# fernandezdaniel/MOBOCMF

Hardware: AMD Instinct MI355X
Metric: ELBO steps/sec (MFDGP d=8 M=512 N=8192 S=8) (higher is better)
Workload: dtype f64

## Files before the change

include/mobocmf_hip.h:

```cpp
#ifndef MOBOCMF_HIP_H
#define MOBOCMF_HIP_H

#include <stddef.h>
#include <stdint.h>

#ifdef __cplusplus
extern "C" {
#endif

typedef void* mobocmf_stream_t;

#define MOBOCMF_MAX_D 32
#define MOBOCMF_MAX_XDIV 48

enum {
    MOBOCMF_OK = 0,
    MOBOCMF_BAD_ARG = 1,
    MOBOCMF_WORKSPACE_TOO_SMALL = 2,
    MOBOCMF_HIP_ERROR = 3,
    MOBOCMF_NOT_PD = 4,
    MOBOCMF_BAD_ARCH = 5
};

typedef struct mobocmf_tuning {
    uint32_t struct_size;
    int32_t small_gemm_max;
    int32_t small_panel_max;
    int32_t tile_rows;
    int32_t pair_mode;
    int32_t mid_gemm_max;
    int32_t mid_gemm_waves;
    int32_t syrk_workgroups;
    int32_t sparse_backward;
    int32_t potrf_cols;
} mobocmf_tuning;
int mobocmf_tuning_init(mobocmf_tuning* t);

typedef struct {
    int32_t kind;
    int32_t d;
    int32_t M;
    int32_t xdiv;
    int64_t Np;
    int32_t branch;
    int32_t want_dx;
    double jitter;
    double min_var;
    int32_t params_const;
    int32_t reserved;
    const mobocmf_tuning* tuning;
    void* const* probe_events;
} mobocmf_layer_desc;
#define MOBOCMF_PROBE_EVENTS 11


int mobocmf_version(void);
int mobocmf_device_arch_ok(void);

int mobocmf_layer_workspace_bytes(const mobocmf_layer_desc* desc, size_t* saved_bytes, size_t* scratch_bytes);

int mobocmf_layer_forward(const mobocmf_layer_desc* desc, const double* x, const double* f, const double* Zx,
                          const double* zf, const double* hyp, const double* m, const double* L_S ,
                          double* mean, double* var, double* kl, int32_t* info, void* saved, size_t saved_bytes,
                          void* scratch, size_t scratch_bytes, mobocmf_stream_t stream);

int mobocmf_layer_backward(const mobocmf_layer_desc* desc, const double* x, const double* f, const double* Zx,
                           const double* zf, const double* hyp, const double* m, const double* L_S,
// ... 402 lines not shown
```

mobocmf_amd/_lib.py:

```python
import ctypes
import os

_HERE = os.path.dirname(os.path.abspath(__file__))
LIB_PATH = os.environ.get("MOBOCMF_HIP_LIB") or os.path.join(_HERE, "csrc", "libmobocmf_hip.so")

OK, BAD_ARG, WORKSPACE_TOO_SMALL, HIP_ERROR, NOT_PD, BAD_ARCH = range(6)
_ERR = {1: "MOBOCMF_BAD_ARG", 2: "MOBOCMF_WORKSPACE_TOO_SMALL", 3: "MOBOCMF_HIP_ERROR", 4: "MOBOCMF_NOT_PD",
        5: "MOBOCMF_BAD_ARCH"}


class Tuning(ctypes.Structure):
    _fields_ = [("struct_size", ctypes.c_uint32), ("small_gemm_max", ctypes.c_int32), ("small_panel_max", ctypes.c_int32),
                ("tile_rows", ctypes.c_int32), ("pair_mode", ctypes.c_int32), ("mid_gemm_max", ctypes.c_int32),
                ("mid_gemm_waves", ctypes.c_int32), ("syrk_workgroups", ctypes.c_int32), ("sparse_backward", ctypes.c_int32),
                ("potrf_cols", ctypes.c_int32)]
    KNOBS = tuple(n for n, _ in _fields_[1:])

    def copy(self):
        t = Tuning()
        ctypes.memmove(ctypes.byref(t), ctypes.byref(self), ctypes.sizeof(Tuning))
        return t


PROBE_EVENTS = 11


class LayerDesc(ctypes.Structure):
    _fields_ = [("kind", ctypes.c_int32), ("d", ctypes.c_int32), ("M", ctypes.c_int32), ("xdiv", ctypes.c_int32),
                ("Np", ctypes.c_int64), ("branch", ctypes.c_int32), ("want_dx", ctypes.c_int32),
                ("jitter", ctypes.c_double), ("min_var", ctypes.c_double), ("params_const", ctypes.c_int32),
                ("reserved", ctypes.c_int32), ("tuning", ctypes.POINTER(Tuning)), ("probe_events", ctypes.c_void_p)]


TINY_MAX_LAYERS, TINY_MAX_M, TINY_MAX_D = 3, 32, 8
COOP_MAX_M = 128
FROZEN_MAX_M = 512
FROZEN_SPLIT_MAX_M = 1024
STEP_GRADIENTS, STEP_UPDATE, STEP_FORWARD, STEP_INPUT_GRADIENTS, STEP_COUPLED = range(5)
STEP_CHAIN_VALID = 16


class TinyModel(ctypes.Structure):
    _L = TINY_MAX_LAYERS
    _fields_ = [("L", ctypes.c_int32), ("M", ctypes.c_int32), ("d", ctypes.c_int32), ("S", ctypes.c_int32),
                ("N", ctypes.c_int32), ("rows", ctypes.c_int32 * _L), ("trainable", ctypes.c_uint32 * _L),
                ("branch", ctypes.c_int32),
                ("x", ctypes.c_void_p), ("y", ctypes.c_void_p), ("fid", ctypes.c_void_p), ("Zx", ctypes.c_void_p),
                ("raw", (ctypes.c_void_p * 7) * _L), ("m", ctypes.c_void_p * _L), ("L_S", ctypes.c_void_p * _L),
                ("raw_noise", ctypes.c_void_p * _L), ("noise_lo", ctypes.c_double * _L), ("noise_hi", ctypes.c_double * _L),
# ... 229 lines not shown
```

mobocmf_amd/csrc/api.hip:

```cpp
#include "common.h"

static const mobocmf_tuning kDefaultTuning = {(uint32_t)sizeof(mobocmf_tuning), 384, 512, 0, 0, 1024, 32, 0, 1, 0};
static thread_local const mobocmf_tuning* t_tuning = nullptr;
static thread_local void* const* t_probe = nullptr;
const mobocmf_tuning& tune() { return t_tuning ? *t_tuning : kDefaultTuning; }
bool tuning_ok(const mobocmf_tuning* t) {
    if (!t) return true;
    return t->struct_size == sizeof(mobocmf_tuning) && t->small_gemm_max >= 1 && t->small_gemm_max <= 512 &&
           t->small_panel_max >= 1 && t->small_panel_max <= 512 && (t->tile_rows == 0 || t->tile_rows == 64 || t->tile_rows == 128) &&
           t->pair_mode >= 0 && t->pair_mode <= 2 && t->mid_gemm_max >= 0 && t->mid_gemm_max <= 4096 &&
           (t->mid_gemm_waves == 4 || t->mid_gemm_waves == 8 || t->mid_gemm_waves == 32) &&
           (t->syrk_workgroups == 0 || (t->syrk_workgroups >= 16 && t->syrk_workgroups <= 4096)) &&
           (t->sparse_backward == 0 || t->sparse_backward == 1) && (t->potrf_cols == 0 || t->potrf_cols == 1 || t->potrf_cols == 4);
}
TuneScope::TuneScope(const mobocmf_tuning* t, void* const* probe) : prev_t(t_tuning), prev_p(t_probe) {
    t_tuning = t;
    t_probe = probe;
}
TuneScope::~TuneScope() {
    t_tuning = prev_t;
    t_probe = prev_p;
}
void probe_at(int i, hipStream_t s) {
    if (t_probe && i < MOBOCMF_PROBE_EVENTS && t_probe[i]) (void)hipEventRecord((hipEvent_t)t_probe[i], s);
}
static void set_pairing(GemmArgs& g) { g.pair_mode = tune().pair_mode; }
static int panel_tile_rows(int, int64_t) { return tune().tile_rows; }

#define TRY(x)              \
    do {                    \
        int _rc = (x);      \
        if (_rc) return _rc; \
    } while (0)

namespace {

struct Bump {
    uintptr_t base;
    size_t off, cap;
    bool ok;
    Bump(void* p, size_t c) : base((uintptr_t)p), off(0), cap(c), ok(true) {}
    double* take(int64_t n) {
        size_t bytes = ((size_t)n * sizeof(double) + 255) & ~(size_t)255;
        if (bytes > cap || off > cap - bytes) { ok = false; off += bytes; return nullptr; }
        double* r = base ? (double*)(base + off) : nullptr;
        off += bytes;
// ... 137 lines not shown
    S.a = b.take(D.Mp); S.mp = b.take(D.Mp);
}
void carve_panel_saved(Bump& b, const Dims& D, PanelSaved& S) {
    int64_t mn = (int64_t)D.Mp * D.Np;
    S.A = b.take(mn); S.C = b.take(mn);
    S.knn = b.take(D.Np); S.q = b.take(D.Np); S.r = b.take(D.Np); S.varraw = b.take(D.Np);
}
void carve_chain_fwd(Bump& b, const Dims& D, ChainWs& S) {
    S.Dinv = b.take((int64_t)(D.Mp / NB) * NB * NB);
    S.Ld = b.take((int64_t)(D.Mp / NB) * NB * NB);
    S.T = b.take((int64_t)D.Mp * D.Mp);
    S.ws_elems = (int64_t)16 * D.Mp * D.Mp;
    S.ws = b.take(S.ws_elems);
    S.klpart = b.take(D.Mp);
}
void carve_panel_fwd(Bump& b, const Dims& D, PanelFwd& S) {
    S.K = b.take((int64_t)D.Mp * D.Np);
    S.qpart = b.take((int64_t)4 * D.nrb * D.Np);
    S.mupart = b.take((int64_t)4 * D.nrb * D.Np);
    S.rpart = b.take((int64_t)4 * D.nrb * D.Np);
}
void carve_chain_bwd_in(Bump& b, const Dims& D, ChainWs& S) {
    int64_t mm = (int64_t)D.Mp * D.Mp;
    S.H = b.take(mm); S.Hc = b.take(mm); S.da = b.take(D.Mp);
}
void carve_chain_bwd(Bump& b, const Dims& D, ChainWs& S) {
    int64_t mm = (int64_t)D.Mp * D.Mp;
    for (int i = 0; i < 8; ++i) S.W[i] = b.take(mm);
    S.da_tot = b.take(D.Mp);
    S.hyp_part2 = b.take((int64_t)D.ggrid_mm.x * D.ggrid_mm.y * hyp_len(1, MOBOCMF_MAX_D));
    S.df_part2 = b.take((int64_t)D.ggrid_mm.y * D.Mp);
    S.dzf_part2 = b.take((int64_t)D.ggrid_mm.x * D.Mp);
}
void carve_panel_bwd(Bump& b, const Dims& D, const mobocmf_layer_desc* d, PanelBwd& S) {
    int64_t mm = (int64_t)D.Mp * D.Mp, mn = (int64_t)D.Mp * D.Np;
    S.gmu = b.take(D.Np); S.gv = b.take(D.Np); S.gv2 = b.take(D.Np); S.cgv = b.take(D.Np);
    S.blkact = (int32_t*)b.take((D.Np / TILE + 1) / 2);
    S.nclamped = (int32_t*)b.take(4);
    S.dA = b.take(mn); S.dK = b.take(mn);
    S.slab_elems = syrk_slab_elems(D.Mp, D.Np);
    S.slabs = b.take(S.slab_elems);
    S.slabs2 = d->branch == 0 ? b.take(S.slab_elems) : nullptr;
    S.dapart = b.take((D.Np <= 8192 ? D.Np / 16 : D.Np / 64) * (int64_t)D.Mp);
    S.hyp_part = b.take((int64_t)D.ggrid_mn.x * D.ggrid_mn.y * D.H);
    S.df_part = S.dzf_part = nullptr;
    if (d->kind == 1) {
        S.df_part = b.take((int64_t)D.ggrid_mn.y * D.Np);
        S.dzf_part = b.take((int64_t)D.ggrid_mn.x * D.Mp);
    }
    S.dx_part = d->want_dx ? b.take((int64_t)D.ggrid_mn.y * D.nbase * d->d) : nullptr;
}

bool carve_single_saved(void* saved, size_t bytes, const Dims& D, ChainWs& c, PanelSaved& p, size_t* used = nullptr) {
    Bump b(saved, bytes);
    carve_chain_state(b, D, c);
    carve_panel_saved(b, D, p);
    if (used) *used = b.off;
    return b.ok;
}
bool carve_single_fwd(void* scratch, size_t bytes, const Dims& D, ChainWs& c, PanelFwd& p, size_t* used = nullptr) {
    Bump b(scratch, bytes);
    carve_chain_fwd(b, D, c);
    carve_panel_fwd(b, D, p);
    if (used) *used = b.off;
    return b.ok;
}
bool carve_single_bwd(void* scratch, size_t bytes, const Dims& D, const mobocmf_layer_desc* d, ChainWs& c, PanelBwd& p,
                      size_t* used = nullptr) {
    Bump b(scratch, bytes);
    carve_panel_bwd(b, D, d, p);
    carve_chain_bwd_in(b, D, c);
    carve_chain_bwd(b, D, c);
    c.slabs = p.slabs;
    c.slab_elems = p.slab_elems;
    if (used) *used = b.off;
    return b.ok;
}
// ... 97 lines not shown
    return MOBOCMF_OK;
}

int panel_backward(const mobocmf_layer_desc* desc, const Dims& D, const ChainWs& c, const PanelSaved& P, const PanelBwd& B,
                   const double* x, const double* f, const double* Zx, const double* zf, const double* hyp, const double* g_mean,
                   const double* g_var, double* g_f, double* g_zf, double* g_hyp, double* g_x, hipStream_t s) {
    const int Mp = D.Mp;
    const int64_t Np = D.Np, mm = (int64_t)Mp * Mp;
    int32_t* nclamped = c.nclamped ? c.nclamped : B.nclamped;
    double* Hc = desc->branch != 0 ? c.H : c.Hc;
    const int32_t* act = tune().sparse_backward ? B.blkact : nullptr;
    TRY(launch_moments_bwd_prep(g_mean, g_var, P.knn, P.q, P.varraw, desc->branch, desc->min_var, D.N, Np, B.gmu, B.gv,
                                B.gv2, B.cgv, nclamped, c.nclamped ? 1 : 0, (int32_t*)act, s));
    int da_parts = 0;
    {
        GemmArgs ga = gemm_args(c.U, Mp, P.C, Np, B.dA, Np, Mp, Np, Mp, TRI_LOWER_A, 2.0);
        ga.bscale = B.gv; ga.epi = EPI_DA; ga.avec = c.a; ga.gmu = B.gmu; ga.cgv = B.cgv; ga.Aaux = P.A;
        ga.Kreal = D.M;
        ga.rowdot_part = desc->params_const ? nullptr : B.dapart;
        ga.colact = act;
        ga.rm = panel_tile_rows(Mp, Np);
        set_pairing(ga);
        probe_at(3, s);
        TRY(launch_gemm(ga, false, 1, s));
        probe_at(4, s);
        da_parts = desc->params_const ? 0 : gemm_rowdot_parts(ga);
    }
    if (!desc->params_const) {
        probe_at(5, s);
        if (desc->branch == 0) TRY(weighted_syrk_pair(P.A, Np, B.gv, B.cgv, Mp, Np, B.slabs, B.slabs2, c.H, Hc, nclamped, act, s));
        else TRY(weighted_syrk(P.A, Np, B.gv, Mp, Np, B.slabs, c.H, nullptr, nullptr, act, s));
        probe_at(6, s);
    }
    {
        GemmArgs ga = gemm_args(c.LinvT, Mp, B.dA, Np, B.dK, Np, Mp, Np, Mp, TRI_UPPER_A, 1.0);
        ga.Kreal = D.M;
        ga.rm = panel_tile_rows(Mp, Np);
        set_pairing(ga);
        ga.colact = act;
        probe_at(7, s);
        TRY(launch_gemm(ga, false, 1, s));
        probe_at(8, s);
    }
    GramArgs g = {};
    g.kind = desc->kind; g.d = desc->d; g.zdiv = 1; g.Zx = Zx; g.zf = zf; g.M = D.M; g.hyp = hyp; g.Mp = Mp;
    g.xdiv = desc->xdiv; g.x = x; g.f = f; g.nbase = D.nbase;
    g.ldk = Np; g.Np = Np; g.G = B.dK; g.gknn = B.cgv; g.colact = act;
    g.hyp_part = B.hyp_part; g.df_part = B.df_part; g.dzf_part = B.dzf_part; g.dx_part = B.dx_part;
    TRY(launch_gram_bwd(g, desc->want_dx != 0, s));
    probe_at(10, s);
    SumTask tk[5];
    int nt = 0;
    if (da_parts > 0) tk[nt++] = {B.dapart, da_parts, Mp, nullptr, 0, 0, c.da, Mp, 0};
    tk[nt++] = {B.hyp_part, (int64_t)D.ggrid_mn.x * D.ggrid_mn.y, D.H, nullptr, 0, 0, g_hyp, D.H, 0};
    if (desc->kind == 1) {
        tk[nt++] = {B.df_part, D.ggrid_mn.y, Np, nullptr, 0, 0, g_f, D.N, 0};
        tk[nt++] = {B.dzf_part, D.ggrid_mn.x, Mp, nullptr, 0, 0, g_zf, D.M, 0};
    }
    if (desc->want_dx)
        tk[nt++] = {B.dx_part, D.ggrid_mn.y, D.nbase * desc->d, nullptr, 0, 0, g_x, D.nbase * desc->d, 0};
    return launch_sum_partials_multi(tk, nt, s);
}

int chain_backward(int n, const ChainWs& c, int64_t zs, const ChainIO& io, const Dims& D, const bool* zero, const int* acc,
                   const bool* fold, hipStream_t s) {
    const int Mp = D.Mp;
    const int64_t mm = (int64_t)Mp * Mp;
    double *G1 = c.W[0], *G2 = c.W[1], *X = c.W[2], *dU = c.W[3], *Y = c.W[4], *T1 = c.W[5], *T2 = c.W[6], *LT = c.W[7];
    double *dL = G1, *T4 = G2, *Gm = X;
    bool any_clamp_branch = false;
    for (int z = 0; z < n; ++z) {
        if (zero[z]) {
            TRY(launch_zero32(c.H + z * zs, mm * 2, s));
            TRY(launch_zero32(c.Hc + z * zs, mm * 2, s));
            TRY(launch_zero32(c.da + z * zs, (int64_t)Mp * 2, s));
        }
        any_clamp_branch = any_clamp_branch || io.desc[z]->branch == 0;
    }
    for (int z = 0; z < n; ++z)
        if (io.desc[z]->branch != 0 && !zero[z] && (n > 1 || any_clamp_branch))
            TRY(launch_copy_block(c.H + z * zs, Mp, c.Hc + z * zs, Mp, Mp, Mp, s));
    const double* Hc = (n == 1 && io.desc[0]->branch != 0) ? c.H : c.Hc;
    {
        GemmArgs g1 = gemm_args(c.UT, Mp, c.H, Mp, G1, Mp, Mp, Mp, Mp, TRI_UPPER_A, 1.0);
        g1.Kreal = D.M;
        TRY(chain_gemm(g1, false, c, n, zs, s));
        GemmArgs g2 = gemm_args(c.U, Mp, G1, Mp, G2, Mp, Mp, Mp, Mp, TRI_LOWER_A, 1.0);
// ... 748 lines not shown
```

mobocmf_amd/csrc/common.h:

```cpp
#pragma once
#include <hip/hip_runtime.h>
#include <stdint.h>

#include "../../include/mobocmf_hip.h"

#define TILE 128
#define NB 64

static inline int64_t round_up(int64_t v, int64_t m) { return (v + m - 1) / m * m; }

#define HIP_TRY(expr)                                   \
    do {                                                \
        hipError_t _e = (expr);                         \
        if (_e != hipSuccess) return MOBOCMF_HIP_ERROR; \
    } while (0)

const mobocmf_tuning& tune();
bool tuning_ok(const mobocmf_tuning* t);
void probe_at(int i, hipStream_t s);
struct TuneScope {
    const mobocmf_tuning* prev_t;
    void* const* prev_p;
    explicit TuneScope(const mobocmf_tuning* t, void* const* probe = nullptr);
    ~TuneScope();
    TuneScope(const TuneScope&) = delete;
    TuneScope& operator=(const TuneScope&) = delete;
};

enum { TRI_NONE = 0, TRI_LOWER_A = 1, TRI_UPPER_A = 2, TRI_LOWER_B = 4, TRI_UPPER_B = 8 };
enum { EPI_STORE = 0, EPI_COLSTATS = 1, EPI_DA = 2 };

struct GemmArgs {
    const double* A;
    const double* B;
    double* C;
    int64_t lda, ldb, ldc;
    int Mr;
    int64_t Nc;
    int64_t Kd;
    int tri;
    int lower_out;
    int sym_out;
    int sym_full;
    int splitk_diag;
    double alpha;
    int accumulate;
    int rm;
    int pair_mode;
    int64_t slab_stride;
    int64_t strideA, strideB, strideC;
    int batched;
    int zlayers;
    int64_t zsA, zsB, zsC;
    const double* bscale;
    int64_t Kreal;
    double* rowdot_part;
    int stream_out;
    const int32_t* skip_if_zero;
    const int32_t* dual_flag;
    const double* bscale2;
    double* C2;
    const int32_t* colact;
    const int32_t* kact;
    int epi;
    double* colsq_part;
    double* coldot_part;
    const double* avec;
    const double* gmu;
    const double* cgv;
    const double* Aaux;
};

int launch_gemm(const GemmArgs& g, bool B_T, int splitk, hipStream_t s);
int gemm_nt_slabs(const GemmArgs& g, int splitk);
bool gemm_nt_is_small(const GemmArgs& g);
int gemm_rowdot_parts(const GemmArgs& g);
int gemm_colstat_rows(const GemmArgs& g);
int launch_gemm_auto(const GemmArgs& g, bool B_T, double* ws, int64_t ws_elems, hipStream_t s);
int launch_gemm_auto_pair(const GemmArgs& a, const GemmArgs& b, double* ws, int64_t ws_elems, hipStream_t s);

#define MAX_ZL 4

struct GramArgs {
    int kind, d, xdiv, zdiv;
    const double* x;
    const double* f;
    int64_t nbase;
    const double* Zx;
    const double* zf;
    int M;
    const double* hyp;
    double* K;
    int64_t ldk;
    int Mp;
    int64_t Np;
    double* knn;
    double jitter;
    int is_kmm;
    int gm;
    const double* G;
    const double* gknn;
    double* hyp_part;
    double* df_part;
    double* dzf_part;
    double* dx_part;
    const int32_t* colact;
};
int launch_gram_fwd(const GramArgs& g, hipStream_t s);
int launch_gram_bwd(const GramArgs& g, bool want_dx, hipStream_t s);
void gram_grid(const GramArgs& g, dim3* grid);
// ... 97 lines not shown
```

mobocmf_amd/csrc/gemm_f64.hip:

```cpp
#include "common.h"
#include <type_traits>
#include <atomic>

typedef double v4f64 __attribute__((ext_vector_type(4)));
typedef double v2f64 __attribute__((ext_vector_type(2)));

#define BM 128
#define BN 128
#define BK 16
#define KL_MAX 1024
#define TILE_ELEMS (BM * BK)

#define IMG_SWZ(row) ((((row) >> 1) & 1) | ((((row) >> 3) & 1) << 2))


template <int CTRL>
__device__ __forceinline__ double dpp_mov(double v) {
    int lo = __double2loint(v), hi = __double2hiint(v);
    lo = __builtin_amdgcn_update_dpp(0, lo, CTRL, 0xF, 0xF, false);
    hi = __builtin_amdgcn_update_dpp(0, hi, CTRL, 0xF, 0xF, false);
    return __hiloint2double(hi, lo);
}
__device__ __forceinline__ double row16_sum(double v) {
    v += dpp_mov<0xB1>(v);
// ... 146 lines not shown
    const double* B = g.B;
    double* C = g.C;
    if (g.batched) {
        const int zl = g.zlayers > 1 ? z % g.zlayers : 0;
        const int zb = g.zlayers > 1 ? z / g.zlayers : z;
        A += zb * g.strideA + zl * g.zsA;
        B += zb * g.strideB + zl * g.zsB;
        C += zb * g.strideC + zl * g.zsC;
    }
    if (!g.batched && splitk > 1) {
        C += z * g.slab_stride;
        if (g.zlayers > 1) {
            A += blockIdx.z * g.zsA;
            B += blockIdx.z * g.zsB;
            C += blockIdx.z * g.zsC;
        }
    }
    const int nparts = (pair && rb != nrb - 1 - rb) ? 2 : 1;
    const int rb_first = rb;

    const int tid = threadIdx.x;
    const int lane = tid & 63;
    const int wave = __builtin_amdgcn_readfirstlane(tid >> 6);
    const int wr = wave >> 1, wc = wave & 1;
    const int li = lane & 15, lk = lane >> 4;

    if constexpr (!B_T) {
        if (g.colact && g.colact[cb] == 0) {
            if (EPI == EPI_DA && g.rowdot_part) {
                for (int part = 0; part < nparts; ++part) {
                    const int rbp = part == 0 ? rb_first : nrb - 1 - rb_first;
                    for (int i = tid; i < 2 * RM; i += 256)
                        g.rowdot_part[((int64_t)cb * 2 + i / RM) * g.Mr + (int64_t)rbp * RM + i % RM] = 0.0;
                }
            }
            return;
        }
    }

    const int a_row = tid >> 3;
    const int a_lchk = (tid & 7) ^ IMG_SWZ(a_row);
    const double* Ag0 = A + (int64_t)a_row * g.lda + a_lchk * 2;
    const double* Bg = B_T ? B + (cb * BN + a_row) * g.ldb + a_lchk * 2
                           : B + (int64_t)wave * g.ldb + cb * BN;
    auto stage = [&](const double* Ag, int64_t k, int buf) {
        double* As = lds + buf * STAGE_ELEMS;
        double* Bs = As + A_ELEMS;
#pragma unroll
        for (int r = 0; r < RM / 32; ++r) glds16(Ag + (int64_t)(32 * r) * g.lda + k, As + (r * 4 + wave) * 128);
        if (B_T) {
#pragma unroll
            for (int r = 0; r < 4; ++r) glds16(Bg + (int64_t)(32 * r) * g.ldb + k, Bs + (r * 4 + wave) * 128);
        } else {
#pragma unroll
            for (int r = 0; r < 4; ++r)
                glds16(Bg + (k + 4 * r) * g.ldb + lane * 2, Bs + (r * 4 + wave) * 128);
        }
    };

    const int swA = IMG_SWZ(li);
    const int colP0 = ((2 * lk + 0) ^ swA) << 1, colP1 = ((2 * lk + 1) ^ swA) << 1;
    const int a_base = (wr * 16 + li) * BK;
    const int bt_base = (wc * 16 + li) * BK;
    const int bn_base = (4 * lk) * BN + wc * 64 + 2 * li;

  STEP_STAMPS_DECL
// ... 211 lines not shown
        bool done = false;
        if constexpr (B_T) {
            if (g.sym_out && g.lower_out && rb == cb) {
                const int wave_u = __builtin_amdgcn_readfirstlane(wave);
                if (wave_u == 1) {
                    STAGE_LOOP(0, nk, 0, KSTEP_LT)
                } else {
                    STAGE_LOOP(0, nk, 0, KSTEP_LE)
                }
                done = true;
            }
        }
        if (!done) { STAGE_LOOP(0, nk, 0, KSTEP_STD(MMA_ALL)) }
    }
#undef STAGE_LOOP
#undef KSTEP
#undef KOFF
#undef KSTEP_STD
#undef STAGE_NEXT
#undef KSTEP_LE
#undef KSTEP_LT
#undef MMA_IF
#undef MMA_ALL
#undef LOAD_A16
#undef LOAD_B16
#undef MMA16

    STAMP(4 + 4 * part);

    const int64_t row0 = (int64_t)rb * RM + wr * 16 + lk;
    const int64_t col0 = cb * BN + (B_T ? wc * 16 + li : wc * 64 + 2 * li);
    const int ccol = B_T ? wc * 16 + li : wc * 64 + 2 * li;
#define COLOFF(nt) (B_T ? (nt) * 32 : ((nt) >> 1) * 32 + ((nt) & 1))
    if (EPI == EPI_DA && !B_T) {
        v2f64 gm[2], cg[2], cs[2];
#pragma unroll
        for (int h = 0; h < 2; ++h) {
            gm[h] = *(const v2f64*)(g.gmu + col0 + 32 * h);
            cg[h] = *(const v2f64*)(g.cgv + col0 + 32 * h);
            cs[h] = (v2f64){1.0, 1.0};
        }
        if (g.bscale) {
#pragma unroll
            for (int h = 0; h < 2; ++h) cs[h] = *(const v2f64*)(g.bscale + col0 + 32 * h);
        }
        double rdkeep = 0.0;
#pragma unroll
        for (int mt = 0; mt < MT; ++mt) {
            v2f64 av[2][4];
            double ar[4];
#pragma unroll
            for (int r = 0; r < 4; ++r) {
                ar[r] = g.avec[row0 + mt * 32 + 4 * r];
#pragma unroll
                for (int h = 0; h < 2; ++h)
                    av[h][r] = *(const v2f64*)(g.Aaux + (row0 + mt * 32 + 4 * r) * g.ldc + col0 + 32 * h);
            }
#pragma unroll
            for (int r = 0; r < 4; ++r) {
                double rd = 0.0;
#pragma unroll
                for (int h = 0; h < 2; ++h) {
                    const v2f64 a = av[h][r];
                    v2f64 o;
                    o[0] = g.alpha * cs[h][0] * acc[mt][2 * h][r] + ar[r] * gm[h][0] - 2.0 * a[0] * cg[h][0];
                    o[1] = g.alpha * cs[h][1] * acc[mt][2 * h + 1][r] + ar[r] * gm[h][1] - 2.0 * a[1] * cg[h][1];
// ... 96 lines not shown
    if (part == 0) STAMP(13);

#undef COLOFF
    STAMP(9 + part);
  }
  STEP_STAMPS_FLUSH;
}

static bool small_panel_ok(const GemmArgs& g, bool B_T, int splitk);
template <int EPI> static int launch_small_panel(const GemmArgs& g, hipStream_t s);
static bool small_gemm_ok(const GemmArgs& g, bool B_T);
static int launch_small_gemm(const GemmArgs& g, bool B_T, hipStream_t s);

static int tile_rows(const GemmArgs& g, bool B_T, int splitk) {
    if (B_T || splitk > 1 || g.batched || g.lower_out || g.zlayers > 1) return BM;
    if (g.rm == 64 || g.rm == BM) return g.rm;
    if (!(g.tri & (TRI_LOWER_A | TRI_UPPER_A))) return BM;
    const int64_t pairs128 = (int64_t)((g.Mr / BM + 1) / 2) * (g.Nc / BN);
    return pairs128 >= 512 ? BM : 64;
}

int launch_gemm(const GemmArgs& g0, bool B_T, int splitk, hipStream_t s) {
    GemmArgs g = g0;
    if (g.Mr % BM || g.Nc % 16 || g.Kd % BK) return MOBOCMF_BAD_ARG;
    if (B_T || g.batched || splitk > 1) g.colact = nullptr;
    if (g.kact) {
        const int sk_min = (g.lower_out && g.splitk_diag > 0 && g.splitk_diag < splitk) ? g.splitk_diag : splitk;
        const int64_t nb = g.Kd / 128;
        if (!B_T || g.batched || splitk <= 1 || g.zlayers > 1 || g.Kd % 128 || (g.tri & (TRI_LOWER_B | TRI_UPPER_B)) ||
            (nb + sk_min - 1) / sk_min + 2 > KL_MAX)
            g.kact = nullptr;
    }
    if (!B_T && ((g.ldc & 1) || ((uintptr_t)g.C & 15))) return MOBOCMF_BAD_ARG;
    if (small_panel_ok(g, B_T, splitk)) {
        if (g.epi == EPI_COLSTATS) return launch_small_panel<EPI_COLSTATS>(g, s);
        if (g.epi == EPI_DA) return launch_small_panel<EPI_DA>(g, s);
        return launch_small_panel<EPI_STORE>(g, s);
    }
    if (g.Nc % BN) return MOBOCMF_BAD_ARG;
    if (B_T && splitk <= 1 && small_gemm_ok(g, true)) return launch_small_gemm(g, true, s);
    if (!B_T && g.batched > 1 && splitk <= 1 && small_gemm_ok(g, false)) return launch_small_gemm(g, false, s);
    const int rm = tile_rows(g, B_T, splitk);
    int nrb = g.Mr / rm;
    int64_t ncb = g.Nc / BN;
    dim3 grid;
    int pair = 0;
    if (g.batched) {
        grid = dim3((unsigned)(nrb * ncb), 1, (unsigned)(g.batched * (g.zlayers > 1 ? g.zlayers : 1)));
        splitk = 1;
    } else if (splitk > 1) {
        int64_t ntile = g.lower_out ? (int64_t)nrb * (nrb + 1) / 2 : (int64_t)nrb * ncb;
        if (g.lower_out && g.splitk_diag > 0) ntile = 0;
        const int64_t nblk = ntile ? ntile * splitk : (int64_t)nrb * (nrb - 1) / 2 * splitk + (int64_t)nrb * g.splitk_diag;
        grid = dim3((unsigned)(g.dual_flag ? 2 * nblk : nblk), 1, (unsigned)(g.zlayers > 1 ? g.zlayers : 1));
    } else {
        const bool can_pair = (g.tri & (TRI_LOWER_A | TRI_UPPER_A)) && !g.lower_out && nrb > 1;
        if (rm == 64) pair = (can_pair && (int64_t)(nrb / 2) * ncb >= 256) ? 1 : 0;
        else pair = (can_pair && (int64_t)nrb * ncb > 512) ? 1 : 0;
        if (g.pair_mode == 1) pair = 0;
        if (g.pair_mode == 2 && (g.tri & (TRI_LOWER_A | TRI_UPPER_A)) && !g.lower_out && nrb > 1) pair = 1;
        grid = dim3((unsigned)((pair ? (nrb + 1) / 2 : nrb) * ncb), 1, 1);
        splitk = 1;
    }
    const bool tri = (g.tri & (TRI_LOWER_A | TRI_UPPER_A)) != 0 || g.epi == EPI_STORE;
#define LAUNCH(BT, TR, EP, RM_) hipLaunchKernelGGL((gemm_f64_kernel<BT, TR, EP, RM_>), grid, dim3(256), 0, s, g, nrb, ncb, splitk, pair)
    if (B_T) {
        if (g.epi != EPI_STORE) return MOBOCMF_BAD_ARG;
        LAUNCH(true, false, EPI_STORE, 128);
    } else if (rm == 64) {
        if (g.epi == EPI_COLSTATS) LAUNCH(false, true, EPI_COLSTATS, 64);
        else if (g.epi == EPI_DA) LAUNCH(false, true, EPI_DA, 64);
        else LAUNCH(false, true, EPI_STORE, 64);
    } else if (tri) {
        if (g.epi == EPI_COLSTATS) LAUNCH(false, true, EPI_COLSTATS, 128);
        else if (g.epi == EPI_DA) LAUNCH(false, true, EPI_DA, 128);
        else LAUNCH(false, true, EPI_STORE, 128);
    } else {
        if (g.epi == EPI_COLSTATS) LAUNCH(false, false, EPI_COLSTATS, 128);
        else if (g.epi == EPI_DA) LAUNCH(false, false, EPI_DA, 128);
        else LAUNCH(false, false, EPI_STORE, 128);
    }
#undef LAUNCH
    return hipGetLastError() == hipSuccess ? MOBOCMF_OK : MOBOCMF_HIP_ERROR;
}

int gemm_colstat_rows(const GemmArgs& g) {
    if (small_panel_ok(g, false, 1)) return 2 * (g.Mr / BM);
    return 2 * (g.Mr / tile_rows(g, false, 1));
}

__global__ void reduce_slabs_kernel(const double* slabs, int64_t slab_stride, int nslab, double* out, int64_t ld,
                                    int rows, int64_t cols, double scale, int lower_only, int tril, int accumulate,
                                    int64_t zs_slabs, int64_t zs_out) {
    int64_t idx = (int64_t)blockIdx.x * blockDim.x + threadIdx.x;
    if (idx >= (int64_t)rows * cols) return;
    slabs += blockIdx.z * zs_slabs;
    out += blockIdx.z * zs_out;
    int i = (int)(idx / cols);
    int64_t j = idx % cols;
    if (lower_only && (j / TILE) > (i / TILE)) {
        if (tril && !accumulate) out[(int64_t)i * ld + j] = 0.0;
        return;
    }
    double v = 0.0;
    const double* p = slabs + (int64_t)i * cols + j;
    for (int z = 0; z < nslab; ++z) v += p[z * slab_stride];
    v *= scale;
    if (tril && j > i) v = 0.0;
    if (accumulate) v += out[(int64_t)i * ld + j];
    out[(int64_t)i * ld + j] = v;
}

static int small_gemm_limit() { return tune().small_gemm_max; }
static int small_panel_limit() { return tune().small_panel_max; }
template <bool B_T>
__device__ __forceinline__ void small_gemm_body(GemmArgs g, const int bz) {
    constexpr int KC = 128;
    __shared__ double As[16][KC + 1], Bs[KC][17];
    if (g.skip_if_zero && *g.skip_if_zero == 0) return;
    const int tx = threadIdx.x & 15, ty = threadIdx.x >> 4;
    const int64_t r0 = (int64_t)blockIdx.y * 16, c0 = (int64_t)blockIdx.x * 16;
    const bool sym_full = B_T && g.sym_full;
// ... 689 lines not shown
```

mobocmf_amd/functional.py:

```python
import contextlib
import ctypes
import os
import threading

import torch

from . import _lib
from ._lib import LayerDesc

JITTER = 1e-6
MIN_VARIANCE = 1e-10

_scratch = {}


def _stream():
    return ctypes.c_void_p(torch.cuda.current_stream().cuda_stream)


def _ptr(t):
    return ctypes.c_void_p(0 if t is None else t.data_ptr())


def _prep(t):
# ... 52 lines not shown
def release_scratch(stream=None):
    if stream is None:
        _scratch.clear()
        return
    for key in [k for k in _scratch if k[1] == stream.cuda_stream]:
        del _scratch[key]


def hyp_len(kind, d):
    return 1 + d if kind == 0 else 5 + 2 * d


_TUNING_DEFAULT = None
_tuning_tls = threading.local()


def _default_tuning():
    global _TUNING_DEFAULT
    if _TUNING_DEFAULT is None:
        t = _lib.Tuning()
        _lib.check(_lib.load().mobocmf_tuning_init(ctypes.byref(t)), "mobocmf_tuning_init")
        _TUNING_DEFAULT = t
    return _TUNING_DEFAULT


def current_tuning():
    t = getattr(_tuning_tls, "override", None)
    return (t if t is not None else _default_tuning()).copy()


def _set_default(**kw):
    t = _default_tuning()
    for k, v in kw.items():
        assert k in _lib.Tuning.KNOBS, k
        setattr(t, k, int(v))


@contextlib.contextmanager
def tuning(**kw):
    prev = getattr(_tuning_tls, "override", None)
    t = current_tuning()
    for k, v in kw.items():
        if k not in _lib.Tuning.KNOBS:
            raise TypeError("unknown tuning knob %r" % k)
        setattr(t, k, int(v))
    _tuning_tls.override = t
    try:
        yield t
    finally:
        _tuning_tls.override = prev


_probe_tls = threading.local()


@contextlib.contextmanager
def probe_events(table, layer=None):
    prev = getattr(_probe_tls, "cur", None)
    _probe_tls.cur = (table, layer)
    try:
        yield
    finally:
        _probe_tls.cur = prev


def _probe_for(layer):
    cur = getattr(_probe_tls, "cur", None)
    if cur is None or (cur[1] is not None and layer is not None and cur[1] != layer):
        return None
    return cur[0]


def make_desc(kind, d, M, Np, xdiv=1, branch=0, want_dx=False, jitter=JITTER, min_var=MIN_VARIANCE, tune=None,
              probe=None, params_const=False):
    if not 1 <= d <= _lib.MAX_D:
        raise _lib.MobocmfError("mobocmf_amd: a layer takes 1..%d input dimensions (got %d): the Gram kernels keep one "
# ... 1144 lines not shown


def set_syrk_workgroups(n=0):
    if int(n) != 0 and not 16 <= int(n) <= 4096:
        raise _lib.MobocmfError("set_syrk_workgroups: 0 | 16..4096")
    _set_default(syrk_workgroups=n)


def set_sparse_backward(on=True):
    _set_default(sparse_backward=1 if on else 0)


_block_act_tls = threading.local()


def set_block_activity(act=None):
    if act is not None:
        assert act.dtype == torch.int32 and act.is_cuda and act.is_contiguous()
    _block_act_tls.act = act


def set_tile_rows(rows=0, pair_mode=0):
    if int(rows) not in (0, 64, 128) or not 0 <= int(pair_mode) <= 2:
        raise _lib.MobocmfError("set_tile_rows: rows 0 | 64 | 128, pair_mode 0..2")
    _set_default(tile_rows=rows, pair_mode=pair_mode)


def set_potrf_cols(cols=0):
    if int(cols) not in (0, 1, 4):
        raise _lib.MobocmfError("set_potrf_cols: 0 | 1 | 4")
    _set_default(potrf_cols=cols)


def set_tuning(small_gemm_max=0, small_panel_max=0):
    if int(small_gemm_max) > 512 or int(small_panel_max) > 512:
        raise _lib.MobocmfError("set_tuning: the small kernels serve dimensions <= 512")
    if small_gemm_max > 0:
        _set_default(small_gemm_max=small_gemm_max)
    if small_panel_max > 0:
        _set_default(small_panel_max=small_panel_max)


def gemm_f64_epilogue(A, B, C, tri, epi, alpha=1.0, stream_out=False, colsq_part=None, coldot_part=None, avec=None,
                      bscale=None, gmu=None, cgv=None, Aaux=None, rowdot_part=None):
    lib = _lib.require_device()
    A, B = _prep(A), _prep(B)
    Mr, Kd = A.shape
    Nc = B.shape[1]
    snap = current_tuning()
    if epi == 1:
        need = gemm_colstat_rows(Mr, Nc, Kd, tri, tune=snap) * Nc
        for part in (colsq_part, coldot_part):
            if part is not None and part.numel() < need:
                raise _lib.MobocmfError("gemm_f64_epilogue: the partial-statistics buffers need gemm_colstat_rows() = %d rows"
                                        % (need // Nc))
    _lib.check(lib.mobocmf_gemm_f64_epilogue(tri, epi, Mr, Nc, Kd, _ptr(A), A.stride(0), _ptr(B), B.stride(0), _ptr(C),
                                             C.stride(0), alpha, int(stream_out), _ptr(colsq_part), _ptr(coldot_part),
                                             _ptr(avec), _ptr(bscale), _ptr(gmu), _ptr(cgv), _ptr(Aaux), _ptr(rowdot_part),
                                             _ptr(getattr(_block_act_tls, "act", None)), ctypes.byref(snap), _stream()),
               "mobocmf_gemm_f64_epilogue")
    return C


def gram(kind, x1, f1, x2, f2, hyp, xdiv=1, knn=False):
    lib = _lib.require_device()
    with torch.no_grad():
        x1, f1, x2, f2, hyp = (_prep(None if t is None else t.detach()) for t in (x1, f1, x2, f2, hyp))
        n1, nb2, d = x1.shape[0], x2.shape[0], x1.shape[1]
        if not 1 <= int(xdiv) <= _lib.MAX_XDIV:
# ... 619 lines not shown
```

Measured before the change: 1068.

## Fuse RBF Gram backward into the dK GEMM epilogue

Adds an EPI_GRAM0 GEMM epilogue that, while the dK = LinvT·dA tile is still in registers, recomputes the squared-exponential kernel from x and Z and accumulates the amplitude and lengthscale gradient partials per tile. For kind-0 layers with xdiv=1, d<=8 and no dx, this replaces the separate gram-backward kernel. That removes one launch and a full re-read of the Mp×Np dK matrix. In exchange the epilogue does per-element exp and lengthscale work inside the GEMM kernel, which adds register and LDS pressure. It is enabled by default through a new tuning knob.

```diff
diff --git a/include/mobocmf_hip.h b/include/mobocmf_hip.h
--- a/include/mobocmf_hip.h
+++ b/include/mobocmf_hip.h
@@ -33,6 +33,7 @@
     int32_t syrk_workgroups;
     int32_t sparse_backward;
     int32_t potrf_cols;
+    int32_t fused_gram_backward;
 } mobocmf_tuning;
 int mobocmf_tuning_init(mobocmf_tuning* t);
 
diff --git a/mobocmf_amd/_lib.py b/mobocmf_amd/_lib.py
--- a/mobocmf_amd/_lib.py
+++ b/mobocmf_amd/_lib.py
@@ -13,8 +13,9 @@
     _fields_ = [("struct_size", ctypes.c_uint32), ("small_gemm_max", ctypes.c_int32), ("small_panel_max", ctypes.c_int32),
                 ("tile_rows", ctypes.c_int32), ("pair_mode", ctypes.c_int32), ("mid_gemm_max", ctypes.c_int32),
                 ("mid_gemm_waves", ctypes.c_int32), ("syrk_workgroups", ctypes.c_int32), ("sparse_backward", ctypes.c_int32),
-                ("potrf_cols", ctypes.c_int32)]
-    KNOBS = tuple(n for n, _ in _fields_[1:])
+                ("potrf_cols", ctypes.c_int32), ("fused_gram_backward", ctypes.c_int32)]
+    KNOBS = tuple(n for n, _ in _fields_[1:10])
+    ALL_KNOBS = tuple(n for n, _ in _fields_[1:])
 
     def copy(self):
         t = Tuning()
diff --git a/mobocmf_amd/csrc/api.hip b/mobocmf_amd/csrc/api.hip
--- a/mobocmf_amd/csrc/api.hip
+++ b/mobocmf_amd/csrc/api.hip
@@ -1,6 +1,6 @@
 #include "common.h"
 
-static const mobocmf_tuning kDefaultTuning = {(uint32_t)sizeof(mobocmf_tuning), 384, 512, 0, 0, 1024, 32, 0, 1, 0};
+static const mobocmf_tuning kDefaultTuning = {(uint32_t)sizeof(mobocmf_tuning), 384, 512, 0, 0, 1024, 32, 0, 1, 0, 1};
 static thread_local const mobocmf_tuning* t_tuning = nullptr;
 static thread_local void* const* t_probe = nullptr;
 const mobocmf_tuning& tune() { return t_tuning ? *t_tuning : kDefaultTuning; }
@@ -11,7 +11,8 @@
            t->pair_mode >= 0 && t->pair_mode <= 2 && t->mid_gemm_max >= 0 && t->mid_gemm_max <= 4096 &&
            (t->mid_gemm_waves == 4 || t->mid_gemm_waves == 8 || t->mid_gemm_waves == 32) &&
            (t->syrk_workgroups == 0 || (t->syrk_workgroups >= 16 && t->syrk_workgroups <= 4096)) &&
-           (t->sparse_backward == 0 || t->sparse_backward == 1) && (t->potrf_cols == 0 || t->potrf_cols == 1 || t->potrf_cols == 4);
+           (t->sparse_backward == 0 || t->sparse_backward == 1) && (t->potrf_cols == 0 || t->potrf_cols == 1 || t->potrf_cols == 4) &&
+           (t->fused_gram_backward == 0 || t->fused_gram_backward == 1);
 }
 TuneScope::TuneScope(const mobocmf_tuning* t, void* const* probe) : prev_t(t_tuning), prev_p(t_probe) {
     t_tuning = t;
@@ -215,6 +216,9 @@
     S.df_part2 = b.take((int64_t)D.ggrid_mm.y * D.Mp);
     S.dzf_part2 = b.take((int64_t)D.ggrid_mm.x * D.Mp);
 }
+bool gram_bwd_fusable(const mobocmf_layer_desc* d) {
+    return tune().fused_gram_backward != 0 && d->kind == 0 && d->xdiv == 1 && d->d <= 8 && !d->want_dx;
+}
 void carve_panel_bwd(Bump& b, const Dims& D, const mobocmf_layer_desc* d, PanelBwd& S) {
     int64_t mm = (int64_t)D.Mp * D.Mp, mn = (int64_t)D.Mp * D.Np;
     S.gmu = b.take(D.Np); S.gv = b.take(D.Np); S.gv2 = b.take(D.Np); S.cgv = b.take(D.Np);
@@ -225,7 +229,9 @@
     S.slabs = b.take(S.slab_elems);
     S.slabs2 = d->branch == 0 ? b.take(S.slab_elems) : nullptr;
     S.dapart = b.take((D.Np <= 8192 ? D.Np / 16 : D.Np / 64) * (int64_t)D.Mp);
-    S.hyp_part = b.take((int64_t)D.ggrid_mn.x * D.ggrid_mn.y * D.H);
+    int64_t hyp_rows = (int64_t)D.ggrid_mn.x * D.ggrid_mn.y;
+    if (gram_bwd_fusable(d) && hyp_rows < 4 * (int64_t)(D.Mp / 64) * (D.Np / TILE)) hyp_rows = 4 * (int64_t)(D.Mp / 64) * (D.Np / TILE);
+    S.hyp_part = b.take(hyp_rows * D.H);
     S.df_part = S.dzf_part = nullptr;
     if (d->kind == 1) {
         S.df_part = b.take((int64_t)D.ggrid_mn.y * D.Np);
@@ -389,27 +395,37 @@
         else TRY(weighted_syrk(P.A, Np, B.gv, Mp, Np, B.slabs, c.H, nullptr, nullptr, act, s));
         probe_at(6, s);
     }
+    int64_t hyp_rows = (int64_t)D.ggrid_mn.x * D.ggrid_mn.y;
     {
         GemmArgs ga = gemm_args(c.LinvT, Mp, B.dA, Np, B.dK, Np, Mp, Np, Mp, TRI_UPPER_A, 1.0);
         ga.Kreal = D.M;
         ga.rm = panel_tile_rows(Mp, Np);
         set_pairing(ga);
         ga.colact = act;
+        const bool fused = gram_bwd_fusable(desc) && gemm_gram_epilogue_ok(ga);
+        if (fused) {
+            ga.epi = EPI_GRAM0;
+            ga.gr_x = x; ga.gr_Zx = Zx; ga.gr_hyp = hyp; ga.gr_gknn = B.cgv; ga.gr_hyp_part = B.hyp_part;
+            ga.gr_nbase = D.nbase; ga.gr_d = desc->d; ga.gr_M = D.M;
+            hyp_rows = gemm_gram_rows(ga);
+        }
         probe_at(7, s);
         TRY(launch_gemm(ga, false, 1, s));
         probe_at(8, s);
-    }
-    GramArgs g = {};
-    g.kind = desc->kind; g.d = desc->d; g.zdiv = 1; g.Zx = Zx; g.zf = zf; g.M = D.M; g.hyp = hyp; g.Mp = Mp;
-    g.xdiv = desc->xdiv; g.x = x; g.f = f; g.nbase = D.nbase;
-    g.ldk = Np; g.Np = Np; g.G = B.dK; g.gknn = B.cgv; g.colact = act;
-    g.hyp_part = B.hyp_part; g.df_part = B.df_part; g.dzf_part = B.dzf_part; g.dx_part = B.dx_part;
-    TRY(launch_gram_bwd(g, desc->want_dx != 0, s));
+        if (!fused) {
+            GramArgs g = {};
+            g.kind = desc->kind; g.d = desc->d; g.zdiv = 1; g.Zx = Zx; g.zf = zf; g.M = D.M; g.hyp = hyp; g.Mp = Mp;
+            g.xdiv = desc->xdiv; g.x = x; g.f = f; g.nbase = D.nbase;
+            g.ldk = Np; g.Np = Np; g.G = B.dK; g.gknn = B.cgv; g.colact = act;
+            g.hyp_part = B.hyp_part; g.df_part = B.df_part; g.dzf_part = B.dzf_part; g.dx_part = B.dx_part;
+            TRY(launch_gram_bwd(g, desc->want_dx != 0, s));
+        }
+    }
     probe_at(10, s);
     SumTask tk[5];
     int nt = 0;
     if (da_parts > 0) tk[nt++] = {B.dapart, da_parts, Mp, nullptr, 0, 0, c.da, Mp, 0};
-    tk[nt++] = {B.hyp_part, (int64_t)D.ggrid_mn.x * D.ggrid_mn.y, D.H, nullptr, 0, 0, g_hyp, D.H, 0};
+    tk[nt++] = {B.hyp_part, hyp_rows, D.H, nullptr, 0, 0, g_hyp, D.H, 0};
     if (desc->kind == 1) {
         tk[nt++] = {B.df_part, D.ggrid_mn.y, Np, nullptr, 0, 0, g_f, D.N, 0};
         tk[nt++] = {B.dzf_part, D.ggrid_mn.x, Mp, nullptr, 0, 0, g_zf, D.M, 0};
diff --git a/mobocmf_amd/csrc/common.h b/mobocmf_amd/csrc/common.h
--- a/mobocmf_amd/csrc/common.h
+++ b/mobocmf_amd/csrc/common.h
@@ -28,7 +28,7 @@
 };
 
 enum { TRI_NONE = 0, TRI_LOWER_A = 1, TRI_UPPER_A = 2, TRI_LOWER_B = 4, TRI_UPPER_B = 8 };
-enum { EPI_STORE = 0, EPI_COLSTATS = 1, EPI_DA = 2 };
+enum { EPI_STORE = 0, EPI_COLSTATS = 1, EPI_DA = 2, EPI_GRAM0 = 3 };
 
 struct GemmArgs {
     const double* A;
@@ -69,6 +69,13 @@
     const double* gmu;
     const double* cgv;
     const double* Aaux;
+    const double* gr_x;
+    const double* gr_Zx;
+    const double* gr_hyp;
+    const double* gr_gknn;
+    double* gr_hyp_part;
+    int64_t gr_nbase;
+    int gr_d, gr_M;
 };
 
 int launch_gemm(const GemmArgs& g, bool B_T, int splitk, hipStream_t s);
@@ -76,6 +83,8 @@
 bool gemm_nt_is_small(const GemmArgs& g);
 int gemm_rowdot_parts(const GemmArgs& g);
 int gemm_colstat_rows(const GemmArgs& g);
+bool gemm_gram_epilogue_ok(const GemmArgs& g);
+int64_t gemm_gram_rows(const GemmArgs& g);
 int launch_gemm_auto(const GemmArgs& g, bool B_T, double* ws, int64_t ws_elems, hipStream_t s);
 int launch_gemm_auto_pair(const GemmArgs& a, const GemmArgs& b, double* ws, int64_t ws_elems, hipStream_t s);
 
diff --git a/mobocmf_amd/csrc/gemm_f64.hip b/mobocmf_amd/csrc/gemm_f64.hip
--- a/mobocmf_amd/csrc/gemm_f64.hip
+++ b/mobocmf_amd/csrc/gemm_f64.hip
@@ -202,6 +202,13 @@
                     const int rbp = part == 0 ? rb_first : nrb - 1 - rb_first;
                     for (int i = tid; i < 2 * RM; i += 256)
                         g.rowdot_part[((int64_t)cb * 2 + i / RM) * g.Mr + (int64_t)rbp * RM + i % RM] = 0.0;
+                }
+            }
+            if (EPI == EPI_GRAM0) {
+                const int H = 1 + g.gr_d;
+                for (int part = 0; part < nparts; ++part) {
+                    const int rbp = part == 0 ? rb_first : nrb - 1 - rb_first;
+                    for (int i = tid; i < 4 * H; i += 256) g.gr_hyp_part[((int64_t)cb * nrb + rbp) * 4 * H + i] = 0.0;
                 }
             }
             return;
@@ -479,6 +486,88 @@
     const int64_t col0 = cb * BN + (B_T ? wc * 16 + li : wc * 64 + 2 * li);
     const int ccol = B_T ? wc * 16 + li : wc * 64 + 2 * li;
 #define COLOFF(nt) (B_T ? (nt) * 32 : ((nt) >> 1) * 32 + ((nt) & 1))
+    if constexpr (EPI == EPI_GRAM0 && !B_T) {
+        const int d = g.gr_d;
+        const double a1 = g.gr_hyp[0];
+        double il[8], aL[8];
+#pragma unroll
+        for (int k = 0; k < 8; ++k) {
+            const double v = k < d ? 1.0 / g.gr_hyp[1 + (k < d ? k : 0)] : 0.0;
+            il[k] = __hiloint2double(__builtin_amdgcn_readfirstlane(__double2hiint(v)), __builtin_amdgcn_readfirstlane(__double2loint(v)));
+            aL[k] = 0.0;
+        }
+        double* xs = lds + STAGE_ELEMS + wave * (STAGE_ELEMS / 4);
+        double* zs = xs + 512;
+        static_assert(512 + MT * 16 * 8 <= STAGE_ELEMS / 4, "the wavefront's x and inducing rows fit its share of a stage buffer");
+        {
+            const int64_t n = cb * BN + wc * 64 + lane;
+            const double* xp = g.gr_x + (n < g.gr_nbase ? n : g.gr_nbase - 1) * d;
+            asm volatile("" : "+v"(xp));
+#pragma unroll
+            for (int k = 0; k < 8; ++k) xs[k * 64 + lane] = xp[k < d ? k : d - 1];
+        }
+#pragma unroll
+        for (int j = 0; j < MT * 2; ++j) {
+            const int idx = lane + 64 * j, rl = idx >> 3, k = idx & 7;
+            const int64_t m = (int64_t)rb * RM + wr * 16 + (rl >> 4) * 32 + (rl & 15);
+            zs[idx] = g.gr_Zx[(m < g.gr_M ? m : g.gr_M - 1) * d + (k < d ? k : d - 1)];
+        }
+        double s_a1 = 0.0;
+        if (g.gr_gknn && rb == 0 && wr == 0 && lk == 0) {
+#pragma unroll
+            for (int nt = 0; nt < 4; ++nt) {
+                const int64_t n = col0 + COLOFF(nt);
+                if (n < g.gr_nbase) s_a1 += g.gr_gknn[n];
+            }
+        }
+#pragma unroll
+        for (int h = 0; h < 2; ++h) {
+            const double* xq = xs + 32 * h + 2 * li;
+            const bool creal0 = col0 + 32 * h < g.gr_nbase, creal1 = col0 + 32 * h + 1 < g.gr_nbase;
+#pragma unroll
+            for (int mt = 0; mt < MT; ++mt) {
+#pragma unroll
+                for (int r = 0; r < 4; ++r) {
+                    const bool rreal = row0 + mt * 32 + 4 * r < g.gr_M;
+                    const double G0 = rreal && creal0 ? g.alpha * acc[mt][2 * h][r] : 0.0;
+                    const double G1 = rreal && creal1 ? g.alpha * acc[mt][2 * h + 1][r] : 0.0;
+                    const v2f64* zp = (const v2f64*)(zs + (mt * 16 + 4 * r + lk) * 8);
+                    double t0[8], t1[8], d0 = 0.0, d1 = 0.0;
+#pragma unroll
+                    for (int k = 0; k < 8; ++k) {
+                        const v2f64 xv = *(const v2f64*)(xq + k * 64);
+                        const double z = zp[k >> 1][k & 1];
+                        t0[k] = (xv[0] - z) * il[k];
+                        t1[k] = (xv[1] - z) * il[k];
+                        d0 += t0[k] * t0[k];
+                        d1 += t1[k] * t1[k];
+                    }
+                    const double E0 = exp(-0.5 * d0), E1 = exp(-0.5 * d1);
+                    s_a1 += G0 * E0;
+                    s_a1 += G1 * E1;
+                    const double W0 = G0 * a1 * E0, W1 = G1 * a1 * E1;
+#pragma unroll
+                    for (int k = 0; k < 8; ++k) {
+                        aL[k] += W0 * t0[k] * t0[k];
+                        aL[k] += W1 * t1[k] * t1[k];
+                    }
+                    __builtin_amdgcn_sched_barrier(0);
+                }
+            }
+        }
+        s_a1 = rows4_sum(row16_sum(s_a1));
+#pragma unroll
+        for (int k = 0; k < 8; ++k) aL[k] = rows4_sum(row16_sum(aL[k])) * il[k];
+        if (lane == 0) {
+            double* hp = g.gr_hyp_part + (((int64_t)cb * nrb + rb) * 4 + wave) * (1 + d);
+            hp[0] = s_a1;
+#pragma unroll
+            for (int k = 0; k < 8; ++k)
+                if (k < d) hp[1 + k] = aL[k];
+        }
+        STAMP(9 + part);
+        continue;
+    }
     if (EPI == EPI_DA && !B_T) {
         v2f64 gm[2], cg[2], cs[2];
 #pragma unroll
@@ -641,6 +730,7 @@
             g.kact = nullptr;
     }
     if (!B_T && ((g.ldc & 1) || ((uintptr_t)g.C & 15))) return MOBOCMF_BAD_ARG;
+    if (g.epi == EPI_GRAM0 && (B_T || splitk > 1 || !gemm_gram_epilogue_ok(g) || g.gr_d < 1 || g.gr_d > 8 || g.accumulate)) return MOBOCMF_BAD_ARG;
     if (small_panel_ok(g, B_T, splitk)) {
         if (g.epi == EPI_COLSTATS) return launch_small_panel<EPI_COLSTATS>(g, s);
         if (g.epi == EPI_DA) return launch_small_panel<EPI_DA>(g, s);
@@ -671,7 +761,7 @@
         grid = dim3((unsigned)((pair ? (nrb + 1) / 2 : nrb) * ncb), 1, 1);
         splitk = 1;
     }
-    const bool tri = (g.tri & (TRI_LOWER_A | TRI_UPPER_A)) != 0 || g.epi == EPI_STORE;
+    const bool tri = (g.tri & (TRI_LOWER_A | TRI_UPPER_A)) != 0 || g.epi == EPI_STORE || g.epi == EPI_GRAM0;
 #define LAUNCH(BT, TR, EP, RM_) hipLaunchKernelGGL((gemm_f64_kernel<BT, TR, EP, RM_>), grid, dim3(256), 0, s, g, nrb, ncb, splitk, pair)
     if (B_T) {
         if (g.epi != EPI_STORE) return MOBOCMF_BAD_ARG;
@@ -679,10 +769,12 @@
     } else if (rm == 64) {
         if (g.epi == EPI_COLSTATS) LAUNCH(false, true, EPI_COLSTATS, 64);
         else if (g.epi == EPI_DA) LAUNCH(false, true, EPI_DA, 64);
+        else if (g.epi == EPI_GRAM0) LAUNCH(false, true, EPI_GRAM0, 64);
         else LAUNCH(false, true, EPI_STORE, 64);
     } else if (tri) {
         if (g.epi == EPI_COLSTATS) LAUNCH(false, true, EPI_COLSTATS, 128);
         else if (g.epi == EPI_DA) LAUNCH(false, true, EPI_DA, 128);
+        else if (g.epi == EPI_GRAM0) LAUNCH(false, true, EPI_GRAM0, 128);
         else LAUNCH(false, true, EPI_STORE, 128);
     } else {
         if (g.epi == EPI_COLSTATS) LAUNCH(false, false, EPI_COLSTATS, 128);
@@ -697,6 +789,11 @@
     if (small_panel_ok(g, false, 1)) return 2 * (g.Mr / BM);
     return 2 * (g.Mr / tile_rows(g, false, 1));
 }
+
+bool gemm_gram_epilogue_ok(const GemmArgs& g) {
+    return !small_panel_ok(g, false, 1) && !g.batched && !g.lower_out && g.zlayers <= 1 && g.Mr % BM == 0 && g.Nc % BN == 0;
+}
+int64_t gemm_gram_rows(const GemmArgs& g) { return 4 * (int64_t)(g.Mr / tile_rows(g, false, 1)) * (g.Nc / BN); }
 
 __global__ void reduce_slabs_kernel(const double* slabs, int64_t slab_stride, int nslab, double* out, int64_t ld,
                                     int rows, int64_t cols, double scale, int lower_only, int tril, int accumulate,
diff --git a/mobocmf_amd/functional.py b/mobocmf_amd/functional.py
--- a/mobocmf_amd/functional.py
+++ b/mobocmf_amd/functional.py
@@ -108,7 +108,7 @@
 def _set_default(**kw):
     t = _default_tuning()
     for k, v in kw.items():
-        assert k in _lib.Tuning.KNOBS, k
+        assert k in _lib.Tuning.ALL_KNOBS, k
         setattr(t, k, int(v))
 
 
@@ -117,7 +117,7 @@
     prev = getattr(_tuning_tls, "override", None)
     t = current_tuning()
     for k, v in kw.items():
-        if k not in _lib.Tuning.KNOBS:
+        if k not in _lib.Tuning.ALL_KNOBS:
             raise TypeError("unknown tuning knob %r" % k)
         setattr(t, k, int(v))
     _tuning_tls.override = t
@@ -1328,9 +1328,11 @@
     _set_default(potrf_cols=cols)
 
 
-def set_tuning(small_gemm_max=0, small_panel_max=0):
+def set_tuning(small_gemm_max=0, small_panel_max=0, fused_gram_backward=None):
     if int(small_gemm_max) > 512 or int(small_panel_max) > 512:
         raise _lib.MobocmfError("set_tuning: the small kernels serve dimensions <= 512")
+    if fused_gram_backward is not None:
+        _set_default(fused_gram_backward=1 if fused_gram_backward else 0)
     if small_gemm_max > 0:
         _set_default(small_gemm_max=small_gemm_max)
     if small_panel_max > 0:
```

Result: no change. 1069, median of 5 (+0.0%).
